# ekimb/rust-mdbg

Hardware: AMD Instinct MI355X
Metric: Gbases/s ingested to k-min-mer graph (higher is better)
Workload: dtype u64

## Files before the change

### include/mdbg_hip.h

```cpp
#ifndef MDBG_HIP_H
#define MDBG_HIP_H

#include <stddef.h>
#include <stdint.h>

#ifdef __cplusplus
extern "C" {
#endif

#define MDBG_ABI_VERSION 3

enum {
    MDBG_OK = 0,
    MDBG_E_PARAM = -1,
    MDBG_E_ALPHABET = -2,
    MDBG_E_CAPACITY = -3,
    MDBG_E_DEVICE = -4,
    MDBG_E_NOMEM = -5,
    MDBG_E_STATE = -6,
    MDBG_E_IO = -7
};

#define MDBG_MAX_L 255u
#define MDBG_MAX_MINABUND 65535u
// ... 25 lines not shown
    const uint32_t* index;
    const uint16_t* abundance;
    const uint32_t* seqlen;
    const uint16_t* shift;
    const uint64_t* shift_full;
    const uint64_t* src_read;
    const uint64_t* src_start;
    const uint64_t* src_end;
    const uint8_t* reversed;
    uint64_t n_distinct;
    uint64_t n_wrapped;
} mdbg_nodes;

typedef struct mdbg_stats {
    uint64_t n_reads, n_bases, n_minimizers, n_windows, n_distinct, table_capacity;
    uint64_t n_slow_tiles;
    uint64_t n_tiles;
    double ms_sketch, ms_insert, ms_finalize;
    double ms_sketch_tile;
    uint64_t n_sketch_tile_launches;
    uint64_t n_sketch_tile_bases;
    uint64_t tile_bases;
    uint64_t n_link_matches;
    uint64_t reserved[3];
} mdbg_stats;

mdbg_ctx* mdbg_create(const mdbg_params* p, int* err);
void mdbg_destroy(mdbg_ctx* ctx);

int mdbg_ingest_batch(mdbg_ctx* ctx, const uint8_t* bases, const uint64_t* offsets, uint64_t n_reads,
                      uint64_t first_read_ordinal);
int mdbg_ingest_batch_device(mdbg_ctx* ctx, const uint8_t* d_bases, const uint64_t* d_offsets, uint64_t n_reads,
                             uint64_t n_bases, uint64_t first_read_ordinal);

typedef struct mdbg_packed_batch {
    const uint64_t* words;
    const uint64_t* offsets;
    uint64_t n_reads;
    const uint64_t* exc_pos;
    const uint8_t* exc_val;
    uint64_t n_exc;
} mdbg_packed_batch;
int mdbg_ingest_batch_packed(mdbg_ctx* ctx, const mdbg_packed_batch* batch, uint64_t first_read_ordinal);
int mdbg_ingest_batch_packed_device(mdbg_ctx* ctx, const mdbg_packed_batch* batch, uint64_t n_bases, uint64_t first_read_ordinal);
int mdbg_sketch_packed_device(mdbg_ctx* ctx, const mdbg_packed_batch* batch, uint64_t n_bases, uint64_t first_read_ordinal);
int mdbg_pack_device(mdbg_ctx* ctx, const uint8_t* d_bases, uint64_t n_bases, uint64_t* d_words, uint64_t* d_exc_pos,
                     uint8_t* d_exc_val, uint64_t exc_cap, uint64_t* n_exc);
// ... 139 lines not shown
```

### rust_mdbg_amd/api.py

```python
import ctypes as C
import os

import numpy as np

_HERE = os.path.dirname(os.path.abspath(__file__))
_LIB = None

MDBG_OK, MDBG_E_PARAM, MDBG_E_ALPHABET, MDBG_E_CAPACITY, MDBG_E_DEVICE, MDBG_E_NOMEM, MDBG_E_STATE, MDBG_E_IO = 0, -1, -2, -3, -4, -5, -6, -7
FLAG_FORCE_GENERIC = 1
FLAG_KEEP_READS = 2


class MdbgError(RuntimeError):
    def __init__(self, code, msg):
        super().__init__("mdbg error %d: %s" % (code, msg))
        self.code = code


class Params(C.Structure):
    _fields_ = [("k", C.c_uint32), ("l", C.c_uint32), ("density", C.c_double), ("min_abundance", C.c_uint32),
                ("reads_already_hpc", C.c_uint32), ("device", C.c_int32), ("flags", C.c_uint32),
                ("table_capacity_hint", C.c_uint64), ("scheme", C.c_uint32), ("syncmer_s", C.c_uint32), ("reserved", C.c_uint64 * 3)]


class Nodes(C.Structure):
    _fields_ = [("n", C.c_uint64), ("k", C.c_uint32), ("keys", C.POINTER(C.c_uint64)), ("index", C.POINTER(C.c_uint32)),
                ("abundance", C.POINTER(C.c_uint16)), ("seqlen", C.POINTER(C.c_uint32)), ("shift", C.POINTER(C.c_uint16)),
                ("shift_full", C.POINTER(C.c_uint64)), ("src_read", C.POINTER(C.c_uint64)), ("src_start", C.POINTER(C.c_uint64)),
                ("src_end", C.POINTER(C.c_uint64)), ("reversed", C.POINTER(C.c_uint8)), ("n_distinct", C.c_uint64),
                ("n_wrapped", C.c_uint64)]


class Stats(C.Structure):
    _fields_ = [("n_reads", C.c_uint64), ("n_bases", C.c_uint64), ("n_minimizers", C.c_uint64), ("n_windows", C.c_uint64),
                ("n_distinct", C.c_uint64), ("table_capacity", C.c_uint64), ("n_slow_tiles", C.c_uint64), ("n_tiles", C.c_uint64),
                ("ms_sketch", C.c_double), ("ms_insert", C.c_double), ("ms_finalize", C.c_double), ("ms_sketch_tile", C.c_double),
                ("n_sketch_tile_launches", C.c_uint64), ("n_sketch_tile_bases", C.c_uint64), ("tile_bases", C.c_uint64),
                ("n_link_matches", C.c_uint64), ("reserved", C.c_uint64 * 3)]


class RoutedLists(C.Structure):
    _fields_ = [("n_all", C.c_uint64), ("n_solid", C.c_uint64), ("d_first", C.c_void_p), ("d_solid", C.c_void_p), ("d_ath", C.c_void_p),
                ("d_count", C.c_void_p), ("d_slot", C.c_void_p), ("d_idx_all", C.c_void_p), ("counts_all", C.c_uint64 * 64),
                ("counts_solid", C.c_uint64 * 64)]


class SketchStore(C.Structure):
    _fields_ = [("n_minimizers", C.c_uint64), ("n_reads", C.c_uint64), ("d_hashes", C.c_void_p), ("d_positions", C.c_void_p),
                ("d_read_offsets", C.c_void_p)]


class BatchInfo(C.Structure):
    _fields_ = [("store_offset", C.c_uint64), ("n_minimizers", C.c_uint64), ("first_slot", C.c_uint64), ("n_reads", C.c_uint64),
                ("first_read_ordinal", C.c_uint64), ("d_hashes", C.c_void_p), ("d_positions", C.c_void_p), ("d_read_offsets", C.c_void_p)]


class EdgeList(C.Structure):
    _fields_ = [("n", C.c_uint64), ("n1", C.POINTER(C.c_uint32)), ("o1", C.POINTER(C.c_uint8)), ("n2", C.POINTER(C.c_uint32)),
                ("o2", C.POINTER(C.c_uint8)), ("overlap", C.POINTER(C.c_uint32)), ("presimp_removed", C.c_uint64)]


# ... 519 lines not shown
```

### rust_mdbg_amd/csrc/api.inc

```
#include <algorithm>
#include <cstdio>
#include <condition_variable>
#include <cstdlib>
#include <cstring>
#include <ctime>
#include <map>
#include <memory>
#include <mutex>
#include <string>
#include <thread>
#include <vector>

#include "../../include/mdbg_hip.h"
#include "edges.h"
#include "unitigs.h"
#include "simplify.h"
#include "contigs.h"

namespace {


constexpr u64 SLAB_BUDGET = 6ull << 30;

inline FILE* alloc_trace() { static FILE* const f = [] { const char* p = getenv("MDBG_ALLOC_TRACE"); return p ? fopen(p, "a") : (FILE*)nullptr; }(); return f; }
// ... 120 lines not shown
    ~HostRaw() { free(p); }
    bool resize(size_t m) {
        if (m > cap) { free(p); cap = m + m / 8 + 16; p = (T*)malloc(cap * sizeof(T)); if (!p) { cap = n = 0; return false; } }
        n = m; return true;
    }
    void clear() { n = 0; }
    T* data() { return p; }
};

struct mdbg_ctx {
    std::recursive_mutex mu;
    std::mutex err_mu;
    Stage stage[2]; std::mutex stage_mu; std::condition_variable stage_cv;
    mdbg_params P{};
    int dev = 0; hipStream_t stream = nullptr; std::string err; int poisoned = 0;
    u64 scal_seq = 0; bool batchwin_zero = false;
    u64* h_scal = nullptr;
    u64 bound = 0; DevBuf d_t4;
    DevBuf mh, mpos, mread, roff; u64 M = 0; u64 mcap = 0; u32 n_slots = 0;
    u64 h_known = 0;
    u64 slot_end_m = 0;
    u64 pending_m = 0;
    std::vector<Batch> batches; size_t batches_inserted = 0;
    DevBuf bread, tile_recs, slab, n_valid, n_scan, last_read, tile_base, scan_tmp, gran_sum, tile_flags, scalars, phase_dbg, shards;
    u32 slab_cap_min = 0;
    DevBuf tab, mx; u64 cap = 0;
    DevBuf arena, route_out, route_tmp, route_h, route_f; u64 n_records = 0; bool routed = false;
    DevBuf by_maps;
    DevBuf link_ctr;
    DevBuf claim;
    bool claims_ok = false;
    DevBuf bm_first, bm_solid, pre_first, pre_solid, popc_tmp, bt_dev, fin_out, solid_list, fin_order;
    DevBuf bm_local, pre_local, pre_local2;
    HostRaw<u64> h_keys, h_shift_full, h_src_read, h_src_start, h_src_end; HostRaw<u32> h_index, h_seqlen; HostRaw<u16> h_abund, h_shift; HostRaw<u8> h_rev;
    std::vector<u64> so_hash, so_pos, so_off;
    std::vector<u32> q_counts; std::vector<u64> q_off; DevBuf q_dev;
    DevBuf syn_bases, syn_off, syn_lens;
    u64 n_reads = 0, n_bases = 0, n_windows = 0, n_distinct = 0, n_slow_tiles = 0, n_tiles = 0;
    double ms_sketch = 0, ms_insert = 0, ms_finalize = 0;
    hipEvent_t ev0 = nullptr, ev1 = nullptr, ev3 = nullptr;
    bool fin_dirty = false;
    int timing = 2;
    std::vector<u8> bt_sent; const void* bt_sent_at = nullptr;
    u32 own_world = 1, own_rank = 0;
    int (*before_emit)(void* self, FinArgs& F, u64 n_solid) = nullptr; void* before_emit_self = nullptr;
    FinArgs finF{}; u64 fin_words = 0, fin_bits = 0; bool fin_open = false;
    u64 fin_rows_guess = 0;
    std::vector<u8> bt_host;
// ... 302 lines not shown
    { int e = next_slot0(c, c->M, n_reads, &slot0); if (e) return e; }
    double dens2 = 2.0 * c->P.density; if (dens2 > 1.0) dens2 = 1.0; if (dens2 < 0) dens2 = 0;
    u32 slab_cap = 0, gather_tiles = 1;
    {
        const double per_base = sync ? std::min(1.0, std::max(0.0, c->P.density)) / (c->P.syncmer_s ? std::max(1.0, (double)(c->P.l - c->P.syncmer_s + 1) / 2.0) : 1.0) : dens2;
        const double e = (double)tile_bases * per_base; double v = e * 1.25 + 6.0 * sqrt(e) + 32.0; if (v > (double)tile_bases) v = (double)tile_bases; slab_cap = ((u32)v + 7u) & ~7u;
        if (e < 128.0) gather_tiles = (u32)std::max(1.0, std::min(16.0, 256.0 / std::max(e, 1.0)));
    }
    if (slab_cap < c->slab_cap_min) slab_cap = c->slab_cap_min;
    static const u32 cap0_hook = getenv("MDBG_SLAB_CAP0") ? (u32)atoi(getenv("MDBG_SLAB_CAP0")) : 0u;
    static const u64 budget_hook = getenv("MDBG_SLAB_BUDGET_MB") ? (u64)atoll(getenv("MDBG_SLAB_BUDGET_MB")) << 20 : 0ull;
    if (cap0_hook && !c->slab_cap_min) slab_cap = std::max<u32>(8u, cap0_hook & ~7u);
    if (slab_cap > (u32)tile_bases) slab_cap = (u32)tile_bases;
    if (n_tiles_total) {
        HIPCHK(c, c->bread.ensure((n_tiles_total + 2) * 4, 0, s));
        HIPCHK(c, c->tile_recs.ensure(n_tiles_total * sizeof(TileRec), 0, s));
        HIPCHK(c, c->n_valid.ensure(n_tiles_total * 4, 0, s));
        HIPCHK(c, c->n_scan.ensure(n_tiles_total * 4, 0, s));
        HIPCHK(c, c->last_read.ensure(n_tiles_total * 4, 0, s));
        if (in.n_exc) HIPCHK(c, c->tile_flags.ensure(n_tiles_total, 0, s));
    }
    u64 want = c->M + (u64)((double)n_bases * dens2 * 1.15) + 65536;
    const bool phase_dbg = getenv("MDBG_PHASE_TIMING") != nullptr;
    for (int attempt = 0; attempt < 4; ++attempt) {
        { int e = store_ensure(c, want); if (e) return e; }
        const u64 chunk = std::max<u64>(1, std::min<u64>(n_tiles_total ? n_tiles_total : 1, (budget_hook ? budget_hook : SLAB_BUDGET) / ((u64)slab_cap * sizeof(Rec))));
        std::vector<u64> part_end;
        for (u64 t0 = 0; t0 < n_tiles_total; t0 += chunk) part_end.push_back(std::min<u64>(n_tiles_total, t0 + chunk));
        u64 max_part = 0; { u64 t0 = 0; for (u64 e : part_end) { max_part = std::max(max_part, e - t0); t0 = e; } }
        if (n_tiles_total) {
            HIPCHK(c, c->slab.ensure((size_t)chunk * slab_cap * sizeof(Rec), 0, s));
            HIPCHK(c, c->tile_base.ensure((size_t)max_part * 8, 0, s));
            HIPCHK(c, c->scan_tmp.ensure(((size_t)max_part / 1024 + 2) * 8, 0, s));
        }
        u64 init[1] = {c->M};
        STAGE_EVENT(c, c->ev0, s);
        SketchInit init0{};
        init0.zero[0] = scal(c) + SC_ERRFLAG; init0.zero[1] = scal(c) + SC_SLOWTOTAL; init0.zero[2] = scal(c) + SC_OVERMAX; init0.set_p = scal(c) + SC_CARRY; init0.set_v = c->M;
        const bool fused = then_insert && inserted && n_tiles_total && part_end.size() == 1 && !phase_dbg && c->cap && c->own_world <= 1 && !c->lmer_on && !c->routed && !c->pending_m &&
                           c->batches_inserted == c->batches.size() && c->mcap > c->M && c->mcap - c->M <= 2 * (want - c->M) + (1u << 20) &&
                           want - c->M <= (48ull << 20);
        if (fused) init0.zero[3] = scal(c) + SC_BATCHWIN;
        if (!n_tiles_total) {
            ZeroList z{};
            z.p[0] = init0.zero[0]; z.n[0] = 1; z.p[1] = init0.zero[1]; z.n[1] = 1; z.p[2] = init0.zero[2]; z.n[2] = 1; z.set_p = init0.set_p; z.set_v = init0.set_v;
            launch_zero_regions(z, s);
            launch_fill_u64(c->roff.as<u64>() + slot0, n_reads + 1, c->M, s);
        }
        SketchArgs A{};
        A.bases = in.d_bases; A.planes = in.d_planes; A.fmt = in.fmt; A.n_bases = n_bases; A.offsets = d_offsets; A.n_reads = (u32)n_reads;
        A.exc_pos = in.d_exc_pos; A.exc_val = in.d_exc_val; A.n_exc = (u32)in.n_exc;
        A.l = c->P.l; A.hpc = c->P.reads_already_hpc == 0 ? 1u : 0u;
        if (n_tiles_total) {
            A.bread = c->bread.as<u32>(); A.recs = c->tile_recs.as<TileRec>(); A.n_tiles = (u32)n_tiles_total;
            A.slab = c->slab.as<Rec>(); A.slab_cap = slab_cap; A.n_valid = c->n_valid.as<u32>(); A.n_scan = c->n_scan.as<u32>(); A.last_read = c->last_read.as<u32>(); A.over_max = (u32*)(scal(c) + SC_OVERMAX);
            A.t4 = c->d_t4.as<u64>();
            A.tile_flags = in.n_exc ? c->tile_flags.as<u8>() : nullptr;
            A.err_flag = (u32*)(scal(c) + SC_ERRFLAG); A.slow_total = (unsigned long long*)(scal(c) + SC_SLOWTOTAL);
            A.read_base = slot0; A.bound = c->bound; A.btop = (u32)(c->bound >> (64 - BS_B)); A.force_slow = ((c->P.flags & 1u) || c->P.l > (u32)BS_MAX_L) ? 1u : 0u;
            A.dbg = nullptr;
            { const char* sp = getenv("MDBG_STOP_PHASE"); A.stop_phase = sp ? (u32)atoi(sp) : 0u; }
            if (phase_dbg) { HIPCHK(c, c->phase_dbg.ensure((size_t)n_tiles_total * 128, 0, s)); HIPCHK(c, hipMemsetAsync(c->phase_dbg.p, 0, (size_t)n_tiles_total * 128, s)); A.dbg = c->phase_dbg.as<u64>(); }
            const u32 n_gran = (u32)((max_part + SCAN_GRAN - 1) / SCAN_GRAN);
            HIPCHK(c, c->gran_sum.ensure((size_t)n_gran * 8 + 64, 0, s));
            A.block_sum = (unsigned long long*)c->gran_sum.as<u64>();
            init0.zero_arr = c->gran_sum.as<u64>(); init0.zero_arr_n = n_gran;
            launch_bread(d_offsets, (u32)n_reads, n_bases, A.n_tiles, c->bread.as<u32>(), c->tile_recs.as<TileRec>(), init0, s);
            if (in.n_exc) {
                HIPCHK(c, hipMemsetAsync(c->tile_flags.p, 0, n_tiles_total, s));
                launch_tile_flags(in.d_exc_pos, (u32)in.n_exc, A.n_tiles, c->tile_flags.as<u8>(), s);
            }
            if (sync) {
                A.scheme = 1; A.s = c->P.syncmer_s; A.btop = 0;
                const double v = c->P.density * (double)(1ull << (2 * c->P.l));
                A.bound = !(v > 0.0) ? 0 : (v >= 18446744073709551616.0 ? ~0ull : (u64)v);
                A.force_slow = ((c->P.flags & 1u) || c->P.syncmer_s > 13) ? 1u : 0u;
            }
            u64 t0 = 0;
            for (size_t pi = 0; pi < part_end.size(); ++pi) {
                const u32 nt = (u32)(part_end[pi] - t0);
                Rec* const part_slab = c->slab.as<Rec>();
                A.tile0 = (u32)t0; A.slab = part_slab;
                if (pi) HIPCHK(c, hipMemsetAsync(c->gran_sum.p, 0, (size_t)n_gran * 8, s));
                { hipEvent_t tb = next_tile_event(c), te = next_tile_event(c); launch_sketch(A, nt, s, tb, te); }
                GatherArgs G{};
                G.tile0 = (u32)t0; G.n = nt; G.slab = part_slab; G.slab_cap = slab_cap; G.n_valid = A.n_valid; G.n_scan = A.n_scan; G.last_read = A.last_read;
                G.out_hash = c->mh.as<u64>(); G.out_pos = c->mpos.as<u32>(); G.out_read = c->mread.as<u32>(); G.out_cap = c->mcap;
                G.m0 = c->M; G.slot0 = slot0; G.n_reads = (u32)n_reads; G.off = c->roff.as<u64>(); G.last_launch = pi + 1 == part_end.size() ? 1u : 0u;
                G.tiles_per_wave = gather_tiles;
                launch_gather(G, c->scan_tmp.as<u64>(), c->tile_base.as<u64>(), scal(c) + SC_CARRY, s, c->gran_sum.as<u64>());
                c->n_tile_launches += 1;
                t0 = part_end[pi];
            }
            c->n_tile_bases += n_bases;
            if (phase_dbg) {
                std::vector<u64> h((size_t)A.n_tiles * 16);
                (void)hipStreamSynchronize(s);
                (void)hipMemcpy(h.data(), A.dbg, h.size() * 8, hipMemcpyDeviceToHost);
                double ph[7] = {0, 0, 0, 0, 0, 0, 0}, nc = 0, nv = 0; u64 nfast = 0;
                for (u32 t = 0; t < A.n_tiles; ++t) {
                    const u64* q = &h[(size_t)t * 16];
                    if (!q[7]) continue;
                    ++nfast;
                    ph[0] += (double)(q[1] - q[0]); ph[1] += (double)(q[2] - q[1]); ph[2] += (double)(q[3] - q[2]); ph[3] += (double)(q[4] - q[3]);
                    ph[4] += (double)(q[5] - q[4]); ph[5] += (double)(q[7] - q[5]);
                    nc += (double)q[9]; nv += (double)q[10];
                }
                const double n = nfast ? (double)nfast : 1.0;
                fprintf(stderr, "[mdbg phase timing] tiles=%u fast=%llu avg cycles: load=%.0f compact=%.0f hash=%.0f exact=%.0f rank=%.0f write=%.0f ; candidates=%.1f valid=%.1f slab_cap=%u\n",
                        A.n_tiles, (unsigned long long)nfast, ph[0] / n, ph[1] / n, ph[2] / n, ph[3] / n, ph[4] / n, ph[5] / n, nc / n, nv / n, slab_cap);
            }
        }
        STAGE_EVENT(c, c->ev1, s);
        u32* const ins_flags = (u32*)(scal(c) + SC_CAPERR);
        if (fused) {
            launch_count_reserve(c->roff.as<u64>(), slot0, (u32)n_reads, c->P.k, scal(c) + SC_BATCHWIN, (u32*)(scal(c) + SC_DONE), c->shards.as<u64>() + SH_DISTINCT * CTR_SHARDS, scal(c) + SC_NDISTINCT,
                                 c->cap, ins_flags + 1, scal(c) + SC_CARRY, c->mcap, (const u32*)(scal(c) + SC_OVERMAX), s);
            if (!c->ev3) HIPCHK(c, hipEventCreate(&c->ev3));
            launch_insert_windows(table_args(c), c->mh.as<u64>(), c->mread.as<u32>(), c->roff.as<u64>(), c->M, c->mcap, slot0, first_ordinal, scal(c) + SC_NWINDOWS, ins_flags, s, scal(c) + SC_CARRY);
            STAGE_EVENT(c, c->ev3, s);
        }
        u64 sc[SC_N];
        int e = read_scalars(c, sc, false, true); if (e) return e;
        c->ms_sketch += ev_ms(c);
        collect_tile_events(c);
        u64 m_new = sc[SC_CARRY];
        const u32 over = (u32)sc[SC_OVERMAX];
        if (over || m_new > c->mcap) {
            if (over) { slab_cap = std::min<u32>((u32)tile_bases, (over + over / 8 + 15u) & ~7u); c->slab_cap_min = slab_cap; }
            if (m_new > c->mcap) want = m_new + 65536;
            c->n_tile_launches -= part_end.size(); c->n_tile_bases -= n_tiles_total ? n_bases : 0;
            continue;
        }
        if (m_new >= 0xFFFFFFF0ull) return fail(c, MDBG_E_CAPACITY, "more than 2^32 minimizers resident on one device");
        if ((u32)sc[SC_ERRFLAG]) {
            u64 which = ~0ull;
            HIPCHK(c, hipMemcpyAsync(scal(c) + SC_SLOWTOTAL, &which, 8, hipMemcpyHostToDevice, s));
            launch_alphabet_rule(A, (unsigned long long*)(scal(c) + SC_SLOWTOTAL), s);
            HIPCHK(c, hipMemcpyAsync(&which, scal(c) + SC_SLOWTOTAL, 8, hipMemcpyDeviceToHost, s));
            HIPCHK(c, hipStreamSynchronize(s));
            if (which != ~0ull) {
                char buf[160]; snprintf(buf, sizeof buf, "Non-ACGTN nucleotide in read %llu of the batch (ordinal %llu)", (unsigned long long)which, (unsigned long long)(first_ordinal + which));
                return fail(c, MDBG_E_ALPHABET, buf);
            }
        }
        const u64 slow_total = sc[SC_SLOWTOTAL];
        if (c->lmer_on && m_new > c->M) {
            const u32 nb = lmer_filter_blocks(m_new - c->M);
            HIPCHK(c, c->slab.ensure((size_t)nb * 256 * sizeof(Rec), 0, s));
            HIPCHK(c, c->n_valid.ensure((size_t)nb * 4, 0, s)); HIPCHK(c, c->tile_base.ensure((size_t)nb * 8, 0, s)); HIPCHK(c, c->scan_tmp.ensure(((size_t)nb / 1024 + 2) * 8, 0, s));
            LmerFilterArgs L{};
// ... 664 lines not shown
    for (size_t i = mark; i < c->batches.size(); ++i) { c->n_reads -= std::min<u64>(c->n_reads, c->batches[i].n_reads); c->n_bases -= std::min<u64>(c->n_bases, c->batches[i].n_bases); }
    c->batches.resize(mark);
    c->batches_inserted = 0;
    if (mark) { const Batch& b = c->batches.back(); c->M = b.m1; c->n_slots = b.slot0 + b.n_reads; c->slot_end_m = b.m1; }
    else { c->M = 0; c->n_slots = 0; c->slot_end_m = 0; c->own_lists_n = 0; }
    return MDBG_OK;
}

int mdbg_set_timing(mdbg_ctx* c, uint32_t level) {
    if (!c || level > 2) return MDBG_E_PARAM;
    MDBG_LOCK(c);
    c->timing = (int)level;
    return MDBG_OK;
}

int mdbg_get_stats(mdbg_ctx* c, mdbg_stats* o) {
    if (!c || !o) return MDBG_E_PARAM;
    MDBG_LOCK(c);
    memset(o, 0, sizeof *o);
    o->n_reads = c->n_reads; o->n_bases = c->n_bases; o->n_minimizers = c->M; o->n_windows = c->n_windows; o->n_distinct = c->n_distinct;
    o->table_capacity = c->cap; o->n_slow_tiles = c->n_slow_tiles; o->n_tiles = c->n_tiles;
    o->ms_sketch = c->ms_sketch; o->ms_insert = c->ms_insert; o->ms_finalize = c->ms_finalize;
    o->ms_sketch_tile = c->ms_tile; o->n_sketch_tile_launches = c->n_tile_launches; o->n_sketch_tile_bases = c->n_tile_bases;
    o->tile_bases = TILE_STRIDE;
    if (c->link_ctr.p) {
        (void)hipSetDevice(c->dev);
        HIPCHK(c, hipStreamSynchronize(c->stream));
        HIPCHK(c, hipMemcpy(&o->n_link_matches, c->link_ctr.p, 8, hipMemcpyDeviceToHost));
    }
    return MDBG_OK;
}

static int fin_setup(mdbg_ctx* c, FinArgs& F, u64& n_words_out, bool byte_maps = false) {
    hipStream_t s = c->stream;
    c->nodes_ok = false; c->ulist_ok = false;
    F.ath_override = nullptr;
    const u32 k = c->P.k;
        std::vector<Batch> bs = c->batches;
        std::sort(bs.begin(), bs.end(), [](const Batch& a, const Batch& b) { return a.first_ordinal < b.first_ordinal; });
        const u32 nb = (u32)bs.size();
        for (u32 i = 0; i + 1 < nb; ++i)
            if (bs[i].n_reads && bs[i].first_ordinal + bs[i].n_reads > bs[i + 1].first_ordinal) {
                char buf[200]; snprintf(buf, sizeof buf, "read ordinals of two batches overlap: [%llu, +%u) and [%llu, +%u) (first_read_ordinal must be the position of the batch's first record in the whole input)",
                                        (unsigned long long)bs[i].first_ordinal, bs[i].n_reads, (unsigned long long)bs[i + 1].first_ordinal, bs[i + 1].n_reads);
                return fail(c, MDBG_E_PARAM, buf);
            }
        std::vector<u64> fo(nb), rb(nb); std::vector<u32> nr(nb), s0(nb);
// ... 583 lines not shown
```

### rust_mdbg_amd/csrc/sketch.hip

```cpp
#include "mdbg_dev.h"
#include "bs_core.h"

enum { FMT_ASCII = 0, FMT_PLANES = 1 };
constexpr int SCAN_GRAN_LOG = 6, SCAN_GRAN = 1 << SCAN_GRAN_LOG;
struct TileRec;

struct SketchArgs {
    const u8* bases;
    const uint2* planes;
    u32 fmt;
    u64 n_bases;
    const u64* offsets; u32 n_reads;
    const u32* bread;
    const TileRec* recs;
    u32 n_tiles;
    u32 tile0, tile_end;
    Rec* slab; u32 slab_cap;
    u32* n_valid;
    u32* n_scan;
    u32* last_read;
    u32* over_max;
    unsigned long long* block_sum;
    const u64* t4;
    const u8* tile_flags;
    const u64* exc_pos; const u8* exc_val; u32 n_exc;
    u32* err_flag; unsigned long long* slow_total;
    u32 read_base;
    u64 bound; u32 l; u32 hpc; u32 btop;
    u32 scheme, s;
    u32 force_slow;
    u64* dbg;
    u32 stop_phase;
};

__device__ inline u32 find_read(const u64* __restrict__ off, u32 lo, u32 hi, u64 p) {
    while (lo < hi) { u32 mid = lo + ((hi - lo + 1) >> 1); if (off[mid] <= p) lo = mid; else hi = mid - 1; }
    return lo;
}


constexpr int TREC_N = 7;
struct __attribute__((aligned(16))) TileRec { u32 rl, rh; int64_t start0; int32_t rel[TREC_N - 1]; int64_t first_base; };
static_assert(sizeof(TileRec) == 48, "three 16-byte words");
struct SketchInit { u64* zero[4]; u64* set_p; u64 set_v; u64* zero_arr; u32 zero_arr_n; };
__global__ void tile_rec_kernel(const u64* __restrict__ off, u32 n_reads, u64 n_bases, u32 n_tiles, u32* __restrict__ bread, TileRec* __restrict__ recs, SketchInit init,
                                int64_t stride, int64_t halo) {
    const u32 t = blockIdx.x * blockDim.x + threadIdx.x;
    if (t == 0) { for (int i = 0; i < 4; ++i) if (init.zero[i]) *init.zero[i] = 0; if (init.set_p) *init.set_p = init.set_v; }
    if (t < init.zero_arr_n) init.zero_arr[t] = 0;
    if (t >= n_tiles + 2) return;
    auto first_pos = [&](u32 e) -> u64 {
        int64_t p = (int64_t)e * stride - halo;
        if (p < 0) p = 0;
        if ((u64)p >= n_bases) p = n_bases ? (int64_t)n_bases - 1 : 0;
        return (u64)p;
// ... 139 lines not shown
__device__ inline u32 dpp_wave_shr1(u32 x) {
    return (u32)__builtin_amdgcn_mov_dpp((int)x, 0x138 , 0xF, 0xF, true);
}

__device__ inline u32 lds_fetch_add(u32* p, u32 v) {
    u32 r;
    const u32 addr = (u32)(uintptr_t)(__attribute__((address_space(3))) u32*)p;
    asm volatile("ds_add_rtn_u32 %0, %1, %2\n\ts_waitcnt lgkmcnt(0)" : "=v"(r) : "v"(addr), "v"(v) : "memory");
    return r;
}

__device__ inline void put_rec(const SketchArgs& a, Rec* slab, u32 rank, u64 hash, u32 pos, u32 read) {
    if (rank < a.slab_cap) { Rec r; r.hash = hash; r.pos = pos; r.read = read; slab[rank] = r; }
}
constexpr u32 LAST_NONE = 0xFFFFFFFFu, LAST_IN_SLAB = 0xFFFFFFFEu;
__device__ inline void put_count(const SketchArgs& a, u32 gt, u32 n, bool last_known = false) {
    a.n_valid[gt] = n;
    if (a.block_sum && n) atomicAdd(a.block_sum + ((gt - a.tile0) >> SCAN_GRAN_LOG), (unsigned long long)n);
    if (a.last_read && !(last_known && n)) a.last_read[gt] = n ? LAST_IN_SLAB : LAST_NONE;
    if (a.n_scan) a.n_scan[gt] = 0;
    if (n > a.slab_cap) atomicMax(a.over_max, n);
}

template <bool HPC, class Src>
__device__ void slow_tile(const SketchArgs& a, const Src& src, u32 gt, Rec* slab, TileLds& S) {
    constexpr int TT = TILE_THREADS;
    const int tid = threadIdx.x % TT;
    const u64 t_lo = (u64)gt * TILE_STRIDE;
    u64 t_hi = t_lo + TILE_STRIDE; if (t_hi > a.n_bases) t_hi = a.n_bases;
    const u32 rl = a.bread[gt], rh_ = a.bread[gt + 2];
    const u64 first_base = a.offsets[0];
    u32* tmp = S.misc;
    if (tid == 0) atomicAdd(a.slow_total, 1ull);
    u32 running = 0;
    for (u64 p0 = t_lo; p0 < t_hi; p0 += TT) {
        const u64 p = p0 + tid;
        u32 sel = 0; u64 hash = 0, start = 0; u32 r = 0; u64 rlo = 0;
        if (p < t_hi && p >= first_base) {
            r = find_read(a.offsets, rl, rh_, p);
            rlo = a.offsets[r];
            const u8 c = src.at(p);
            if (c != 'A' && c != 'C' && c != 'G' && c != 'T' && c != 'N') *a.err_flag = 1;
            if (kept_at<HPC>(src, rlo, p) && walk_lmer<HPC>(src, rlo, p, a.l, start, hash) && hash <= a.bound) sel = 1;
        }
        u32 total;
        const u32 rank = tile_excl_scan(sel, tmp, total);
        if (sel) put_rec(a, slab, running + rank, hash, (u32)(start - rlo), r + a.read_base);
        running += total;
    }
    if (tid == 0) put_count(a, gt, running);
}

constexpr int SYNC_KEEP = 8;
__device__ inline u64 sync_hash(u64 key, u64 mask) {
    key = (~key + (key << 21)) & mask;
    key = key ^ key >> 24;
    key = ((key + (key << 3)) + (key << 8)) & mask;
    key = key ^ key >> 14;
    key = ((key + (key << 2)) + (key << 4)) & mask;
    key = key ^ key >> 28;
    key = (key + (key << 31)) & mask;
    return key;
}
__device__ inline u32 sync_hash32(u32 key, u32 mask) {
    key = (~key + (key << 21)) & mask;
    key = key ^ key >> 24;
    key = ((key + (key << 3)) + (key << 8)) & mask;
    key = key ^ key >> 14;
    key = ((key + (key << 2)) + (key << 4)) & mask;
    key = key ^ key >> 28;
    key = (key + (key << 31)) & mask;
    return key;
}
// ... 84 lines not shown
                        for (u32 j = 1; j < l; ++j) {
                            u64 q2 = st - 1;
                            if (HPC) { const u8 c2 = src.at(q2); if (in_hpc_set(c2)) while (q2 > rlo && src.at(q2 - 1) == c2) --q2; }
                            st = q2;
                        }
                        Rec rec; rec.hash = hl; rec.pos = (u32)(st - rlo); rec.read = rr + a.read_base;
                        if (write) { if (base + n_mine < a.slab_cap) slab[base + n_mine] = rec; }
                        else if (n_mine < SYNC_KEEP) keep[n_mine] = rec;
                        ++n_mine;
                    }
                }
            }
            if (!restart) break;
            n_mine = 0;
        }
    };
    run(false, 0);
    if (n_mine > SYNC_KEEP) any_over = 1;
    u32 total;
    const u32 base = block_excl_scan_256(n_mine, sc_tmp, total);
    if (!any_over) {
        for (u32 i = 0; i < n_mine; ++i) if (base + i < a.slab_cap) slab[base + i] = keep[i];
    } else run(true, base);
    if (tid == 0) put_count(a, gt, total);
}


struct CandOut { u64 hash; u32 pos, read; };

#define MDBG_HOT(cond, value) (cond)
template <int L, int SCHEME = 0, int WMAX = 1>
__global__ __launch_bounds__(TILE_THREADS, SCHEME ? 5 : 6) void sketch_bs_kernel(SketchArgs a) {
    constexpr int TT = TILE_THREADS, RW = TILE_RAW_WORDS, HW = TILE_HW, QCAP = TILE_QCAP, RS_CAP = TILE_RS_CAP, STAGE_AT = TILE_STAGE_AT;
    __shared__ TileLdsS<SCHEME> S;
    __shared__ __attribute__((aligned(16))) u64 S_t3[T3_WORDS];
    __shared__ u32 sync_tmp[SCHEME ? 16 : 1];
    const u32 Lr = SCHEME ? a.l : (u32)L;
    const int tid = (int)threadIdx.x, lane = tid & 63, wv = tid >> 6;
    const int64_t nb = (int64_t)a.n_bases;
    const int64_t n_pairs = (nb + 31) >> 5;
    const bool hpc = MDBG_HOT(a.hpc != 0, true);
    typedef u32 u32x4 __attribute__((ext_vector_type(4)));
    const u32 wg = blockIdx.x, gt = a.tile0 + wg;
    Rec* const slab = a.slab + (size_t)wg * a.slab_cap;
#define MDBG_STAMP(i) do { if (a.dbg && tid == 0) a.dbg[(size_t)gt * 16 + (i)] = __builtin_readcyclecounter(); } while (0)
    MDBG_STAMP(0);
    const int64_t raw0 = (int64_t)gt * TILE_STRIDE - TILE_HALO;
// ... 564 lines not shown
                if (j < n) { e = S.c.list[j]; h = exact(e); pass = h <= a.bound; if (!pass) clear_bit(e); }
                const u64 bal = __ballot(pass);
                if (bal) {
                    u32 base = 0;
                    if (lane == 0) base = atomicAdd(&S.misc[18 + i], (u32)__popcll(bal));
                    base = (u32)__builtin_amdgcn_readfirstlane((int)base);
                    if (pass) { const u32 slot = base + __builtin_amdgcn_mbcnt_hi((u32)(bal >> 32), __builtin_amdgcn_mbcnt_lo((u32)bal, 0u)); S.c.surv[slot] = (u16)e; s_h[slot] = h; }
                }
                __syncthreads();
                const u32 n_surv = S.misc[18 + i];
                if ((u32)tid < n_surv) {
                    e = S.c.surv[tid];
                    keep_e[i] = e;
                    if (place(e, s_h[tid], keep[i])) keep_ok |= 1u << i; else clear_bit(e);
                }
            }
        }
        __syncthreads();
        MDBG_STAMP(4);
        if (MDBG_HOT(a.stop_phase == 4, false)) return 0u;
        const u32 left = count_words();
        MDBG_STAMP(5);
        if (MDBG_HOT(a.stop_phase == 5, false)) return 0u;
#pragma unroll
        for (int i = 0; i < NR; ++i) if ((keep_ok >> i) & 1u) {
            const u32 rank = rank_of(keep_e[i]);
            put_rec(a, slab, rank, keep[i].hash, keep[i].pos, keep[i].read);
            if (rank + 1 == left && a.last_read) a.last_read[gt] = keep[i].read;
        }
        return left;
    };

    const u32 n_cand = S.misc[17];
    if (MDBG_HOT(n_cand <= QCAP, true)) {
        const u32 nv = n_cand ? process_list(n_cand) : 0;
        if (tid == 0) { put_count(a, gt, nv, true); if (a.dbg) { a.dbg[(size_t)gt * 16 + 9] = n_cand; a.dbg[(size_t)gt * 16 + 10] = nv; } }
    } else {
        __syncthreads();
        if constexpr (SCHEME == 1) {
            {
                const uint4 cw = *(const uint4*)(S.c.cand + WPT * tid);
                u32 w5[5] = {cw.x, cw.y, cw.z, cw.w, tid == TT - 1 ? S.c.cand[RW] : 0u};
#pragma unroll
                for (int i = 0; i < 5; ++i) {
                    u32 w = w5[i], keep = w;
                    while (w) {
                        const u32 b = (u32)__clz(w), bit = 0x80000000u >> b; w &= ~bit;
                        if (exact((u32)(32 * (WPT * tid + i)) + b - (BS_B - 1)) > a.bound) keep &= ~bit;
                    }
                    w5[i] = keep;
                }
                *(uint4*)(S.c.cand + WPT * tid) = make_uint4(w5[0], w5[1], w5[2], w5[3]);
                if (tid == TT - 1) S.c.cand[RW] = w5[4];
                if (tid == 0) S.misc[17] = 0;
            }
            __syncthreads();
            expand_list();
            __syncthreads();
            const u32 n2 = S.misc[17];
            if (n2 <= QCAP) {
                const u32 nv = n2 ? process_list(n2) : 0;
                if (tid == 0) { put_count(a, gt, nv, true); if (a.dbg) { a.dbg[(size_t)gt * 16 + 9] = n_cand; a.dbg[(size_t)gt * 16 + 10] = nv; } }
                return;
            }
            __syncthreads();
        }
        const u32 C = count_words();
        const u32 per = (C + TT - 1) / TT;
        const u32 r0 = (u32)tid * per < C ? (u32)tid * per : C, r1 = r0 + per < C ? r0 + per : C;
        u32 surv = 0;
        if (r0 < r1) {
            u32 lo = 0, hi = RW;
            while (lo < hi) { const u32 mid = (lo + hi + 1) >> 1; if (S.c.cpre[mid] <= r0) lo = mid; else hi = mid - 1; }
            u32 D = lo, w = S.c.cand[D];
            for (u32 skip = r0 - S.c.cpre[D]; skip; --skip) w &= ~(0x80000000u >> (u32)__clz(w));
            for (u32 r = r0; r < r1; ++r) {
                while (!w) { ++D; w = S.c.cand[D]; }
                const u32 b = (u32)__clz(w); w &= ~(0x80000000u >> b);
                const u32 e = 32 * D + b - (BS_B - 1);
                const u64 h = exact(e);
                CandOut o{}; bool ok = false;
                if (h <= a.bound) ok = place(e, h, o);
                Rec rec; rec.hash = ok ? o.hash : 0ull; rec.pos = ok ? o.pos : 0u; rec.read = ok ? o.read : 0xFFFFFFFFu;
                surv += ok ? 1u : 0u;
                if (r < a.slab_cap) slab[r] = rec;
            }
        }
        u32 nv;
        tile_excl_scan(surv, S.misc, nv);
        if (tid == 0) {
            a.n_valid[gt] = nv; if (a.n_scan) a.n_scan[gt] = C;
            if (a.block_sum && nv) atomicAdd(a.block_sum + ((gt - a.tile0) >> SCAN_GRAN_LOG), (unsigned long long)nv);
            if (a.last_read) a.last_read[gt] = nv ? LAST_IN_SLAB : LAST_NONE;
            if (C > a.slab_cap) atomicMax(a.over_max, C);
            if (a.dbg) { a.dbg[(size_t)gt * 16 + 9] = n_cand; a.dbg[(size_t)gt * 16 + 10] = nv; }
        }
    }
    MDBG_STAMP(7);
#undef MDBG_STAMP
}

__global__ __launch_bounds__(256) void tile_scan_sums_kernel(u32 n, const u32* __restrict__ n_valid, u64* __restrict__ block_sum) {
    __shared__ u32 ws[4];
    const u32 i0 = blockIdx.x * 1024 + threadIdx.x * 4;
    u32 v = 0;
#pragma unroll
    for (int q = 0; q < 4; ++q) if (i0 + q < n) v += n_valid[i0 + q];
    for (int d = 32; d; d >>= 1) v += __shfl_down(v, d, 64);
    if ((threadIdx.x & 63) == 0) ws[threadIdx.x >> 6] = v;
    __syncthreads();
    if (threadIdx.x == 0) block_sum[blockIdx.x] = (u64)ws[0] + ws[1] + ws[2] + ws[3];
}
__global__ __launch_bounds__(256) void tile_scan_top_kernel(u32 n_blocks, u64* __restrict__ block_sum, u64* __restrict__ carry) {
// ... 173 lines not shown
        const Rec r = cur;
        if (j0 + 64 < S) cur = fetch(j0 + 64 + lane);
        const bool valid = r.read != REC_REJECTED;
        const u64 bal = __ballot(valid);
        const u64 lower = bal & ((1ull << lane) - 1ull);
        const u32 from_lane = __shfl(r.read, lower ? 63 - __clzll((long long)lower) : 0, 64);
        const int64_t pr = lower ? (int64_t)from_lane : prev;
        const u32 last_valid = __shfl(r.read, bal ? 63 - __clzll((long long)bal) : 0, 64);
        if (valid) {
            const u64 idx = out + (u64)__popcll(lower);
            if (idx < g.out_cap) { g.out_hash[idx] = r.hash; g.out_pos[idx] = r.pos; g.out_read[idx] = r.read; }
            int64_t c = (int64_t)r.read; if (c > hi) c = hi;
            for (int64_t x = pr + 1; x <= c; ++x) g.off[x] = idx;
        }
        if (bal) prev = (int64_t)last_valid;
        out += (u64)__popcll(bal);
    }
    if (tail) {
        int64_t last = prev < lo ? lo : prev;
        for (int64_t x = last + 1 + lane; x <= hi; x += 64) g.off[x] = out;
    }
}

template <class Src>
__global__ __launch_bounds__(256) void alphabet_rule_kernel(Src src, const u64* __restrict__ off, u32 n_reads, u32 l, u32 hpc,
                                                            unsigned long long* __restrict__ which) {
    const u32 r = blockIdx.x * 4 + (threadIdx.x >> 6);
    if (r >= n_reads) return;
    const u32 lane = threadIdx.x & 63;
    const u64 a = off[r], b = off[r + 1];
    u64 kept = 0; bool bad = false;
    for (u64 p = a + lane; p < b; p += 64) {
        const u8 c = src.at(p);
        bad |= !(c == 'A' || c == 'C' || c == 'G' || c == 'T' || c == 'N');
        if (!hpc || p == a || !(c == src.at(p - 1) && in_hpc_set(c))) ++kept;
    }
    for (int d = 32; d; d >>= 1) kept += __shfl_down(kept, d, 64);
    const bool any_bad = __ballot(bad) != 0;
    if (lane == 0 && any_bad && kept >= l) atomicMin(which, (unsigned long long)r);
}

__global__ void tile_flags_kernel(const u64* __restrict__ exc_pos, u32 n_exc, u32 n_tiles, u8* __restrict__ flags, u64 stride, u64 halo) {
    const u32 i = blockIdx.x * blockDim.x + threadIdx.x;
    if (i >= n_exc) return;
    const u64 p = exc_pos[i];
    const u64 t = p / stride;
// ... 161 lines not shown
```

Before: 2533.

## Write sketch output directly via decoupled look-back tile chaining

After: 1961. 22.6% lower.

```diff
diff --git a/include/mdbg_hip.h b/include/mdbg_hip.h
--- a/include/mdbg_hip.h
+++ b/include/mdbg_hip.h
@@ -71,7 +71,8 @@
     uint64_t n_sketch_tile_bases;
     uint64_t tile_bases;
     uint64_t n_link_matches;
-    uint64_t reserved[3];
+    uint64_t n_direct_fallbacks;
+    uint64_t reserved[2];
 } mdbg_stats;
 
 mdbg_ctx* mdbg_create(const mdbg_params* p, int* err);
diff --git a/rust_mdbg_amd/api.py b/rust_mdbg_amd/api.py
--- a/rust_mdbg_amd/api.py
+++ b/rust_mdbg_amd/api.py
@@ -36,7 +36,7 @@
                 ("n_distinct", C.c_uint64), ("table_capacity", C.c_uint64), ("n_slow_tiles", C.c_uint64), ("n_tiles", C.c_uint64),
                 ("ms_sketch", C.c_double), ("ms_insert", C.c_double), ("ms_finalize", C.c_double), ("ms_sketch_tile", C.c_double),
                 ("n_sketch_tile_launches", C.c_uint64), ("n_sketch_tile_bases", C.c_uint64), ("tile_bases", C.c_uint64),
-                ("n_link_matches", C.c_uint64), ("reserved", C.c_uint64 * 3)]
+                ("n_link_matches", C.c_uint64), ("n_direct_fallbacks", C.c_uint64), ("reserved", C.c_uint64 * 2)]
 
 
 class RoutedLists(C.Structure):
diff --git a/rust_mdbg_amd/csrc/api.inc b/rust_mdbg_amd/csrc/api.inc
--- a/rust_mdbg_amd/csrc/api.inc
+++ b/rust_mdbg_amd/csrc/api.inc
@@ -166,8 +166,10 @@
     u64 slot_end_m = 0;
     u64 pending_m = 0;
     std::vector<Batch> batches; size_t batches_inserted = 0;
-    DevBuf bread, tile_recs, slab, n_valid, n_scan, last_read, tile_base, scan_tmp, gran_sum, tile_flags, scalars, phase_dbg, shards;
+    DevBuf bread, tile_recs, slab, n_valid, n_scan, last_read, tile_base, scan_tmp, gran_sum, tile_status, tile_flags, scalars, phase_dbg, shards;
     u32 slab_cap_min = 0;
+    bool direct_off = false;
+    u64 n_direct_fallbacks = 0;
     DevBuf tab, mx; u64 cap = 0;
     DevBuf arena, route_out, route_tmp, route_h, route_f; u64 n_records = 0; bool routed = false;
     DevBuf by_maps;
@@ -516,7 +518,11 @@
     }
     u64 want = c->M + (u64)((double)n_bases * dens2 * 1.15) + 65536;
     const bool phase_dbg = getenv("MDBG_PHASE_TIMING") != nullptr;
-    for (int attempt = 0; attempt < 4; ++attempt) {
+    static const bool direct_hook = !(getenv("MDBG_SKETCH_DIRECT") && atoi(getenv("MDBG_SKETCH_DIRECT")) == 0);
+    static const u32 polls_hook = getenv("MDBG_LOOKBACK_POLLS") ? (u32)std::max(1, atoi(getenv("MDBG_LOOKBACK_POLLS"))) : (4u << 20);
+    const bool stop_hook = getenv("MDBG_STOP_PHASE") != nullptr;
+    for (int attempt = 0; attempt < 5; ++attempt) {
+        const bool direct = direct_hook && !c->direct_off && !stop_hook;
         { int e = store_ensure(c, want); if (e) return e; }
         const u64 chunk = std::max<u64>(1, std::min<u64>(n_tiles_total ? n_tiles_total : 1, (budget_hook ? budget_hook : SLAB_BUDGET) / ((u64)slab_cap * sizeof(Rec))));
         std::vector<u64> part_end;
@@ -556,9 +562,18 @@
             { const char* sp = getenv("MDBG_STOP_PHASE"); A.stop_phase = sp ? (u32)atoi(sp) : 0u; }
             if (phase_dbg) { HIPCHK(c, c->phase_dbg.ensure((size_t)n_tiles_total * 128, 0, s)); HIPCHK(c, hipMemsetAsync(c->phase_dbg.p, 0, (size_t)n_tiles_total * 128, s)); A.dbg = c->phase_dbg.as<u64>(); }
             const u32 n_gran = (u32)((max_part + SCAN_GRAN - 1) / SCAN_GRAN);
+            const size_t status_bytes = ((size_t)max_part * 8 + 15) & ~(size_t)15;
+            if (direct) {
+                HIPCHK(c, c->tile_status.ensure(status_bytes + 64, 0, s));
+                A.status = c->tile_status.as<u64>(); A.n_scan = nullptr; A.last_read = nullptr; A.block_sum = nullptr;
+                A.out_hash = c->mh.as<u64>(); A.out_pos = c->mpos.as<u32>(); A.out_read = c->mread.as<u32>(); A.out_cap = c->mcap;
+                A.carry = scal(c) + SC_CARRY; A.lb_fail = (u32*)(scal(c) + SC_OVERMAX) + 1; A.poll_limit = polls_hook;
+                init0.zero_arr = c->tile_status.as<u64>(); init0.zero_arr_n = (u32)max_part;
+            } else {
             HIPCHK(c, c->gran_sum.ensure((size_t)n_gran * 8 + 64, 0, s));
             A.block_sum = (unsigned long long*)c->gran_sum.as<u64>();
             init0.zero_arr = c->gran_sum.as<u64>(); init0.zero_arr_n = n_gran;
+            }
             launch_bread(d_offsets, (u32)n_reads, n_bases, A.n_tiles, c->bread.as<u32>(), c->tile_recs.as<TileRec>(), init0, s);
             if (in.n_exc) {
                 HIPCHK(c, hipMemsetAsync(c->tile_flags.p, 0, n_tiles_total, s));
@@ -575,8 +590,12 @@
                 const u32 nt = (u32)(part_end[pi] - t0);
                 Rec* const part_slab = c->slab.as<Rec>();
                 A.tile0 = (u32)t0; A.slab = part_slab;
-                if (pi) HIPCHK(c, hipMemsetAsync(c->gran_sum.p, 0, (size_t)n_gran * 8, s));
+                if (pi) {
+                    if (direct) HIPCHK(c, hipMemsetAsync(c->tile_status.p, 0, status_bytes, s));
+                    else HIPCHK(c, hipMemsetAsync(c->gran_sum.p, 0, (size_t)n_gran * 8, s));
+                }
                 { hipEvent_t tb = next_tile_event(c), te = next_tile_event(c); launch_sketch(A, nt, s, tb, te); }
+                if (direct) { c->n_tile_launches += 1; t0 = part_end[pi]; continue; }
                 GatherArgs G{};
                 G.tile0 = (u32)t0; G.n = nt; G.slab = part_slab; G.slab_cap = slab_cap; G.n_valid = A.n_valid; G.n_scan = A.n_scan; G.last_read = A.last_read;
                 G.out_hash = c->mh.as<u64>(); G.out_pos = c->mpos.as<u32>(); G.out_read = c->mread.as<u32>(); G.out_cap = c->mcap;
@@ -585,6 +604,12 @@
                 launch_gather(G, c->scan_tmp.as<u64>(), c->tile_base.as<u64>(), scal(c) + SC_CARRY, s, c->gran_sum.as<u64>());
                 c->n_tile_launches += 1;
                 t0 = part_end[pi];
+            }
+            if (direct) {
+                ReadOffArgs R{};
+                R.mread = c->mread.as<u32>(); R.m0 = c->M; R.carry = scal(c) + SC_CARRY; R.cap = c->mcap; R.flags = (const u32*)(scal(c) + SC_OVERMAX);
+                R.slot0 = slot0; R.n_reads = (u32)n_reads; R.off = c->roff.as<u64>();
+                launch_read_offsets(R, c->mcap - c->M, s);
             }
             c->n_tile_bases += n_bases;
             if (phase_dbg) {
@@ -598,11 +623,12 @@
                     ++nfast;
                     ph[0] += (double)(q[1] - q[0]); ph[1] += (double)(q[2] - q[1]); ph[2] += (double)(q[3] - q[2]); ph[3] += (double)(q[4] - q[3]);
                     ph[4] += (double)(q[5] - q[4]); ph[5] += (double)(q[7] - q[5]);
+                    if (q[6]) ph[6] += (double)(q[6] - q[5]);
                     nc += (double)q[9]; nv += (double)q[10];
                 }
                 const double n = nfast ? (double)nfast : 1.0;
-                fprintf(stderr, "[mdbg phase timing] tiles=%u fast=%llu avg cycles: load=%.0f compact=%.0f hash=%.0f exact=%.0f rank=%.0f write=%.0f ; candidates=%.1f valid=%.1f slab_cap=%u\n",
-                        A.n_tiles, (unsigned long long)nfast, ph[0] / n, ph[1] / n, ph[2] / n, ph[3] / n, ph[4] / n, ph[5] / n, nc / n, nv / n, slab_cap);
+                fprintf(stderr, "[mdbg phase timing] tiles=%u fast=%llu avg cycles: load=%.0f compact=%.0f hash=%.0f exact=%.0f rank=%.0f write=%.0f (chain=%.0f) ; candidates=%.1f valid=%.1f slab_cap=%u\n",
+                        A.n_tiles, (unsigned long long)nfast, ph[0] / n, ph[1] / n, ph[2] / n, ph[3] / n, ph[4] / n, ph[5] / n, ph[6] / n, nc / n, nv / n, slab_cap);
             }
         }
         STAGE_EVENT(c, c->ev1, s);
@@ -619,8 +645,13 @@
         c->ms_sketch += ev_ms(c);
         collect_tile_events(c);
         u64 m_new = sc[SC_CARRY];
-        const u32 over = (u32)sc[SC_OVERMAX];
-        if (over || m_new > c->mcap) {
+        u32 over = (u32)sc[SC_OVERMAX];
+        if (sc[SC_OVERMAX] >> 32) {
+            c->direct_off = true; c->n_direct_fallbacks += 1;
+            if (over <= slab_cap) over = 0;
+            m_new = c->M;
+        }
+        if ((sc[SC_OVERMAX] >> 32) || over || m_new > c->mcap) {
             if (over) { slab_cap = std::min<u32>((u32)tile_bases, (over + over / 8 + 15u) & ~7u); c->slab_cap_min = slab_cap; }
             if (m_new > c->mcap) want = m_new + 65536;
             c->n_tile_launches -= part_end.size(); c->n_tile_bases -= n_tiles_total ? n_bases : 0;
@@ -1331,7 +1362,7 @@
     o->table_capacity = c->cap; o->n_slow_tiles = c->n_slow_tiles; o->n_tiles = c->n_tiles;
     o->ms_sketch = c->ms_sketch; o->ms_insert = c->ms_insert; o->ms_finalize = c->ms_finalize;
     o->ms_sketch_tile = c->ms_tile; o->n_sketch_tile_launches = c->n_tile_launches; o->n_sketch_tile_bases = c->n_tile_bases;
-    o->tile_bases = TILE_STRIDE;
+    o->tile_bases = TILE_STRIDE; o->n_direct_fallbacks = c->n_direct_fallbacks;
     if (c->link_ctr.p) {
         (void)hipSetDevice(c->dev);
         HIPCHK(c, hipStreamSynchronize(c->stream));
diff --git a/rust_mdbg_amd/csrc/sketch.hip b/rust_mdbg_amd/csrc/sketch.hip
--- a/rust_mdbg_amd/csrc/sketch.hip
+++ b/rust_mdbg_amd/csrc/sketch.hip
@@ -31,6 +31,11 @@
     u32 force_slow;
     u64* dbg;
     u32 stop_phase;
+    u64* status;
+    u64* out_hash; u32* out_pos; u32* out_read; u64 out_cap;
+    u64* carry;
+    u32* lb_fail;
+    u32 poll_limit;
 };
 
 __device__ inline u32 find_read(const u64* __restrict__ off, u32 lo, u32 hi, u64 p) {
@@ -216,6 +221,79 @@
     if (n > a.slab_cap) atomicMax(a.over_max, n);
 }
 
+typedef __attribute__((address_space(1))) u64 gu64;
+constexpr u64 ST_COUNT = 1ull << 62, ST_PREFIX = 2ull << 62, ST_VALUE = (1ull << 62) - 1;
+constexpr u64 CHAIN_FAILED = ~0ull;
+__device__ inline u64 st_load(const u64* p) { return __hip_atomic_load((gu64*)p, __ATOMIC_RELAXED, __HIP_MEMORY_SCOPE_AGENT); }
+__device__ inline void st_store(u64* p, u64 v) { __hip_atomic_store((gu64*)p, v, __ATOMIC_RELAXED, __HIP_MEMORY_SCOPE_AGENT); }
+__device__ inline u64 tile_lookback(const SketchArgs& a, u32 wg, u32 n, int lane) {
+    u64 excl = 0; bool ok = true;
+    if (wg == 0) excl = st_load(a.carry);
+    else {
+        if (lane == 0) st_store(a.status + wg, ST_COUNT | n);
+        int64_t top = (int64_t)wg - 1;
+        for (u32 polls = 0;;) {
+            const int64_t idx = top - lane;
+            u64 w = ST_COUNT;
+            if (idx >= 0) w = st_load(a.status + idx);
+            const u64 bal_p = __ballot((w >> 62) == 2), bal_e = __ballot((w >> 62) == 0);
+            const u32 f = bal_p ? (u32)__builtin_ctzll(bal_p) : 64u;
+            if (bal_e & (f < 64u ? (1ull << f) - 1ull : ~0ull)) {
+                if (++polls >= a.poll_limit) { ok = false; break; }
+                __builtin_amdgcn_s_sleep(2);
+                continue;
+            }
+            excl += (u32)__builtin_amdgcn_readlane((int)wave_incl_scan((u32)lane < f ? (u32)w : 0u), 63);
+            if (bal_p) {
+                const u32 lo = (u32)__builtin_amdgcn_readlane((int)(u32)w, (int)f), hi = (u32)__builtin_amdgcn_readlane((int)(u32)((w & ST_VALUE) >> 32), (int)f);
+                excl += (u64)hi << 32 | lo;
+                break;
+            }
+            top -= 64;
+            if (top < 0) { ok = false; break; }
+        }
+    }
+    if (lane == 0) {
+        if (ok) {
+            st_store(a.status + wg, ST_PREFIX | (excl + n));
+            if (wg + 1 == gridDim.x) st_store(a.carry, excl + n);
+        } else { atomicOr(a.lb_fail, 1u); atomicMax(a.over_max, 1u); }
+    }
+    return ok ? excl : CHAIN_FAILED;
+}
+__device__ inline u64 tile_chain(const SketchArgs& a, u32 wg, u32 n, u32* sh) {
+    if (threadIdx.x < 64) {
+        const u64 b = tile_lookback(a, wg, n, (int)threadIdx.x);
+        if (threadIdx.x == 0) { sh[0] = (u32)b; sh[1] = (u32)(b >> 32); }
+    }
+    __syncthreads();
+    return (u64)(u32)__builtin_amdgcn_readfirstlane((int)sh[1]) << 32 | (u32)__builtin_amdgcn_readfirstlane((int)sh[0]);
+}
+__device__ inline void put_store(const SketchArgs& a, u64 idx, u64 hash, u32 pos, u32 read) {
+    if (idx < a.out_cap) { a.out_hash[idx] = hash; a.out_pos[idx] = pos; a.out_read[idx] = read; }
+}
+__device__ inline void slab_to_store(const SketchArgs& a, u32 wg, const Rec* slab, u32 n, u32 n_slots, u32* sh) {
+    asm volatile("s_waitcnt vmcnt(0)" ::: "memory");
+    const u64 base = tile_chain(a, wg, n, sh + 12);
+    if (n_slots > a.slab_cap) { if (threadIdx.x == 0) atomicMax(a.over_max, n_slots); return; }
+    if (base == CHAIN_FAILED) return;
+    if (n_slots == n) {
+        for (u32 j = threadIdx.x; j < n; j += TILE_THREADS) { const Rec r = slab[j]; put_store(a, base + j, r.hash, r.pos, r.read); }
+    } else {
+        u32 run = 0;
+        for (u32 j0 = 0; j0 < n_slots; j0 += TILE_THREADS) {
+            const u32 j = j0 + threadIdx.x;
+            Rec r{}; r.read = 0xFFFFFFFFu;
+            if (j < n_slots) r = slab[j];
+            const u32 valid = r.read != 0xFFFFFFFFu ? 1u : 0u;
+            u32 total;
+            const u32 rank = block_excl_scan_256(valid, sh, total);
+            if (valid) put_store(a, base + run + rank, r.hash, r.pos, r.read);
+            run += total;
+        }
+    }
+}
+
 template <bool HPC, class Src>
 __device__ void slow_tile(const SketchArgs& a, const Src& src, u32 gt, Rec* slab, TileLds& S) {
     constexpr int TT = TILE_THREADS;
@@ -242,7 +320,8 @@
         if (sel) put_rec(a, slab, running + rank, hash, (u32)(start - rlo), r + a.read_base);
         running += total;
     }
-    if (tid == 0) put_count(a, gt, running);
+    if (a.status) slab_to_store(a, blockIdx.x, slab, running, running, tmp);
+    else if (tid == 0) put_count(a, gt, running);
 }
 
 constexpr int SYNC_KEEP = 8;
@@ -373,7 +452,8 @@
     if (!any_over) {
         for (u32 i = 0; i < n_mine; ++i) if (base + i < a.slab_cap) slab[base + i] = keep[i];
     } else run(true, base);
-    if (tid == 0) put_count(a, gt, total);
+    if (a.status) slab_to_store(a, blockIdx.x, slab, total, total, sc_tmp);
+    else if (tid == 0) put_count(a, gt, total);
 }
 
 
@@ -984,6 +1064,14 @@
         const u32 left = count_words();
         MDBG_STAMP(5);
         if (MDBG_HOT(a.stop_phase == 5, false)) return 0u;
+        if (MDBG_HOT(a.status != nullptr, true)) {
+            const u64 base = tile_chain(a, wg, left, S.misc + 24);
+            MDBG_STAMP(6);
+            if (base == CHAIN_FAILED) return left;
+#pragma unroll
+            for (int i = 0; i < NR; ++i) if ((keep_ok >> i) & 1u) put_store(a, base + rank_of(keep_e[i]), keep[i].hash, keep[i].pos, keep[i].read);
+            return left;
+        }
 #pragma unroll
         for (int i = 0; i < NR; ++i) if ((keep_ok >> i) & 1u) {
             const u32 rank = rank_of(keep_e[i]);
@@ -996,7 +1084,8 @@
     const u32 n_cand = S.misc[17];
     if (MDBG_HOT(n_cand <= QCAP, true)) {
         const u32 nv = n_cand ? process_list(n_cand) : 0;
-        if (tid == 0) { put_count(a, gt, nv, true); if (a.dbg) { a.dbg[(size_t)gt * 16 + 9] = n_cand; a.dbg[(size_t)gt * 16 + 10] = nv; } }
+        if (a.status && !n_cand) (void)tile_chain(a, wg, 0u, S.misc + 24);
+        if (tid == 0) { if (!a.status) put_count(a, gt, nv, true); if (a.dbg) { a.dbg[(size_t)gt * 16 + 9] = n_cand; a.dbg[(size_t)gt * 16 + 10] = nv; } }
     } else {
         __syncthreads();
         if constexpr (SCHEME == 1) {
@@ -1022,7 +1111,8 @@
             const u32 n2 = S.misc[17];
             if (n2 <= QCAP) {
                 const u32 nv = n2 ? process_list(n2) : 0;
-                if (tid == 0) { put_count(a, gt, nv, true); if (a.dbg) { a.dbg[(size_t)gt * 16 + 9] = n_cand; a.dbg[(size_t)gt * 16 + 10] = nv; } }
+                if (a.status && !n2) (void)tile_chain(a, wg, 0u, S.misc + 24);
+                if (tid == 0) { if (!a.status) put_count(a, gt, nv, true); if (a.dbg) { a.dbg[(size_t)gt * 16 + 9] = n_cand; a.dbg[(size_t)gt * 16 + 10] = nv; } }
                 return;
             }
             __syncthreads();
@@ -1050,7 +1140,10 @@
         }
         u32 nv;
         tile_excl_scan(surv, S.misc, nv);
-        if (tid == 0) {
+        if (a.status) {
+            slab_to_store(a, wg, slab, nv, C, S.misc);
+            if (tid == 0 && a.dbg) { a.dbg[(size_t)gt * 16 + 9] = n_cand; a.dbg[(size_t)gt * 16 + 10] = nv; }
+        } else if (tid == 0) {
             a.n_valid[gt] = nv; if (a.n_scan) a.n_scan[gt] = C;
             if (a.block_sum && nv) atomicAdd(a.block_sum + ((gt - a.tile0) >> SCAN_GRAN_LOG), (unsigned long long)nv);
             if (a.last_read) a.last_read[gt] = nv ? LAST_IN_SLAB : LAST_NONE;
@@ -1270,6 +1363,31 @@
     }
 }
 
+struct ReadOffArgs { const u32* mread; u64 m0; const u64* carry; u64 cap; const u32* flags; u32 slot0, n_reads; u64* off; };
+__global__ __launch_bounds__(256) void read_offsets_kernel(ReadOffArgs g) {
+    const u64 m1 = *g.carry;
+    if (m1 > g.cap || m1 < g.m0 || g.flags[0] || g.flags[1]) return;
+    const int64_t lo = (int64_t)g.slot0 - 1, hi = (int64_t)g.slot0 + g.n_reads;
+    const u64 n = m1 - g.m0, stride = (u64)gridDim.x * 256;
+    for (u64 j = (u64)blockIdx.x * 256 + threadIdx.x; j < n; j += stride) {
+        const u64 i = g.m0 + j;
+        int64_t cur = (int64_t)g.mread[i], prev = j ? (int64_t)g.mread[i - 1] : lo;
+        if (cur > hi) cur = hi;
+        if (prev < lo) prev = lo;
+        for (int64_t x = prev + 1; x <= cur; ++x) g.off[x] = i;
+    }
+    if (blockIdx.x == 0) {
+        int64_t last = n ? (int64_t)g.mread[m1 - 1] : lo;
+        if (last < lo) last = lo;
+        for (int64_t x = last + 1 + threadIdx.x; x <= hi; x += 256) g.off[x] = m1;
+    }
+}
+void launch_read_offsets(const ReadOffArgs& g, u64 room, hipStream_t s) {
+    u64 nb = (room + 1023) / 1024;
+    nb = nb < 1 ? 1 : nb > 2048 ? 2048 : nb;
+    hipLaunchKernelGGL(read_offsets_kernel, dim3((unsigned)nb), dim3(256), 0, s, g);
+}
+
 template <class Src>
 __global__ __launch_bounds__(256) void alphabet_rule_kernel(Src src, const u64* __restrict__ off, u32 n_reads, u32 l, u32 hpc,
                                                             unsigned long long* __restrict__ which) {
```
